# mrjoshuak/go-jpeg2000

Measured on AMD Instinct MI355X. Metric: Mpixels/s encode+decode (4K sRGB, 5-3 lossless), higher is better.
Workload: dtype int32

## Files before the change

### go-jpeg2000_amd/csrc/compact.hip

```cpp
#include "j2k_internal.h"
#include <algorithm>

namespace j2k {

template <bool TWO>
__global__ __launch_bounds__(1024) void scan_lens_kernel(const uint32_t *__restrict__ lens, int n, uint64_t *__restrict__ offs,
                                                         const uint32_t *__restrict__ mels, uint64_t *__restrict__ toffs) {
    __shared__ uint64_t wave_sum[2][16], wave_sum2[2][16];
    const int tid = threadIdx.x, lane = tid & 63, wv = tid >> 6;
    uint64_t carry = 0, carry2 = 0;
    int par = 0;
    for (int base = 0; base < n; base += 8192, par ^= 1) {
        const int i0 = base + tid * 8;
        uint32_t v[8], m[8];
        if (i0 + 8 <= n) {
            const uint4 a = *reinterpret_cast<const uint4 *>(lens + i0), b = *reinterpret_cast<const uint4 *>(lens + i0 + 4);
            v[0] = a.x; v[1] = a.y; v[2] = a.z; v[3] = a.w; v[4] = b.x; v[5] = b.y; v[6] = b.z; v[7] = b.w;
        } else {
#pragma unroll
            for (int k = 0; k < 8; k++) v[k] = (i0 + k < n) ? lens[i0 + k] : 0u;
        }
        if (TWO && i0 + 8 <= n) {
            const uint4 a = *reinterpret_cast<const uint4 *>(mels + i0), b = *reinterpret_cast<const uint4 *>(mels + i0 + 4);
            m[0] = a.x; m[1] = a.y; m[2] = a.z; m[3] = a.w; m[4] = b.x; m[5] = b.y; m[6] = b.z; m[7] = b.w;
        } else {
#pragma unroll
            for (int k = 0; k < 8; k++) m[k] = (TWO && i0 + k < n) ? mels[i0 + k] : 0u;
        }
#pragma unroll
        for (int k = 0; k < 8; k++) m[k] = v[k] ? m[k] : 0u;
        uint64_t t = 0, t2 = 0;
#pragma unroll
        for (int k = 0; k < 8; k++) { t += v[k]; if (TWO) t2 += v[k] - m[k]; }
        uint64_t x = t, x2 = t2;
        for (int o = 1; o < 64; o <<= 1) {
            const uint64_t y = __shfl_up(x, o);
            if (lane >= o) x += y;
            if (TWO) {
                const uint64_t y2 = __shfl_up(x2, o);
                if (lane >= o) x2 += y2;
            }
        }
        if (lane == 63) { wave_sum[par][wv] = x; if (TWO) wave_sum2[par][wv] = x2; }
        __syncthreads();
        uint64_t pre = carry, all = carry, pre2 = carry2, all2 = carry2;
#pragma unroll
        for (int k = 0; k < 16; k++) {
            const uint64_t ws = wave_sum[par][k], ws2 = TWO ? wave_sum2[par][k] : 0;
            if (k < wv) { pre += ws; pre2 += ws2; }
            all += ws; all2 += ws2;
        }
        uint64_t o = pre + x - t, o2 = pre2 + x2 - t2;
#pragma unroll
        for (int k = 0; k < 8; k++) {
            if (i0 + k < n) { offs[i0 + k] = o; if (TWO) toffs[i0 + k] = o2; }
            o += v[k]; o2 += v[k] - m[k];
        }
        carry = all; carry2 = all2;
    }
    if (tid == 0) { offs[n] = carry; if (TWO) toffs[n] = carry2; }
}

__global__ __launch_bounds__(256) void gather_kernel(const BlockJob *__restrict__ jobs, int njobs, const uint8_t *__restrict__ slots,
                                                     const uint32_t *__restrict__ lens, const uint64_t *__restrict__ offs,
                                                     uint8_t *__restrict__ stream, const uint32_t *__restrict__ maglens) {
    const int j = blockIdx.x * 4 + (threadIdx.x >> 6);
    if (j >= njobs) return;
    const int lane = threadIdx.x & 63;
    const uint32_t len = lens[j];
    if (len == 0) return;
    gather_job(jobs[j], slots, stream + offs[j], len, maglens != nullptr, maglens ? maglens[j] : 0u, lane);
}

__global__ __launch_bounds__(256) void gather_scan_kernel(const BlockJob *__restrict__ jobs, int njobs, const uint8_t *__restrict__ slots,
                                                          const uint32_t *__restrict__ lens, uint64_t *__restrict__ offs,
                                                          uint8_t *__restrict__ stream, const uint32_t *__restrict__ maglens) {
    __shared__ uint64_t s_wave[4];
    __shared__ uint32_t s_len[4];
    const int tid = threadIdx.x, wv = tid >> 6, lane = tid & 63;
    const int j0 = blockIdx.x * 4, j = j0 + wv;
    const bool mine = j < njobs;
    const uint32_t len = mine ? lens[j] : 0u;
    const uint32_t mag = (mine && maglens) ? maglens[j] : 0u;
    BlockJob J = jobs[mine ? j : 0];
    uint64_t part = 0;
#pragma unroll
    for (int p = 0; p < 8; p++) {
        const int i0 = 1024 * p + 4 * tid;
        if (i0 + 4 <= j0) {
            const uint4 v = *reinterpret_cast<const uint4 *>(lens + i0);
            part += (uint64_t)v.x + v.y + v.z + v.w;
        } else {
#pragma unroll
            for (int i = 0; i < 3; i++)
                if (i0 + i < j0) part += lens[i0 + i];
        }
    }
#pragma unroll
    for (int o = 32; o > 0; o >>= 1) part += __shfl_xor(part, o);
    if (lane == 0) { s_wave[wv] = part; s_len[wv] = len; }
    __syncthreads();
    uint64_t off = s_wave[0] + s_wave[1] + s_wave[2] + s_wave[3];
#pragma unroll
    for (int k = 0; k < 3; k++)
        if (k < wv) off += s_len[k];
    if (!mine) return;
    if (lane == 0) {
        offs[j] = off;
        if (j == njobs - 1) offs[njobs] = off + len;
    }
    if (len == 0) return;
    gather_job(J, slots, stream + off, len, maglens != nullptr, mag, lane);
}

#define UNPACK_BATCH 16
__host__ __device__ inline size_t pack_a16(size_t x) { return (x + 15) & ~size_t(15); }
struct PackLayout { size_t lens, mag, nb, offs, toffs, payload; };
__host__ __device__ inline PackLayout pack_layout(size_t n) {
    PackLayout L;
    L.lens = 64;
    L.mag = pack_a16(L.lens + 4 * n);
    L.nb = pack_a16(L.mag + 4 * n);
    L.offs = pack_a16(L.nb + n);
    L.toffs = pack_a16(L.offs + 8 * (n + 1));
    L.payload = pack_a16(L.toffs + 8 * (n + 1));
    return L;
}
size_t pack_header_bytes(size_t n) { return pack_layout(n).payload; }

__device__ __forceinline__ uint32_t mel_bytes(const BlockJob &J) {
    const size_t nsamp = (size_t)J.w * J.h;
    return (uint32_t)((nsamp * 2 < 64 ? 64 : nsamp * 2) / 4);
}

__global__ __launch_bounds__(256) void pack_kernel(const BlockJob *__restrict__ jobs, int n, const uint8_t *__restrict__ stream,
                                                   const uint64_t *__restrict__ offs, const uint64_t *__restrict__ toffs,
                                                   const uint32_t *__restrict__ lens, const uint32_t *__restrict__ maglens,
                                                   const uint8_t *__restrict__ numbps, uint8_t *__restrict__ pack) {
    const PackLayout L = pack_layout((size_t)n);
    const int has_mel = maglens != nullptr;
    if (blockIdx.x == 0 && threadIdx.x == 0) {
        uint64_t *h = reinterpret_cast<uint64_t *>(pack);
        h[0] = ((uint64_t)L.payload + toffs[n] + 15) & ~uint64_t(15);
        h[1] = toffs[n];
        reinterpret_cast<uint32_t *>(pack)[4] = (uint32_t)n;
        reinterpret_cast<uint32_t *>(pack)[5] = (uint32_t)has_mel;
    }
    const int j = blockIdx.x * 4 + (threadIdx.x >> 6);
    if (j > n) return;
    const int lane = threadIdx.x & 63;
    const uint64_t off = offs[j], toff = toffs[j];
    if (lane == 0) {
        reinterpret_cast<uint64_t *>(pack + L.offs)[j] = off;
        reinterpret_cast<uint64_t *>(pack + L.toffs)[j] = toff;
    }
    if (j == n) return;
    const uint32_t len = lens[j];
    const uint32_t mag = has_mel ? maglens[j] : len;
    if (lane == 0) {
        reinterpret_cast<uint32_t *>(pack + L.lens)[j] = len;
        reinterpret_cast<uint32_t *>(pack + L.mag)[j] = mag;
        pack[L.nb + j] = numbps[j];
    }
    if (len == 0) return;
    const uint32_t mel = has_mel ? mel_bytes(jobs[j]) : 0u;
    const uint8_t *src = stream + off;
    uint8_t *dst = pack + L.payload + toff;
    copy_bytes(dst, src, mag, lane);
    copy_bytes(dst + mag, src + mag + mel, len - mag - mel, lane);
}
__global__ void mel_table_kernel(const BlockJob *__restrict__ jobs, int n, uint32_t *__restrict__ mels) {
    const int j = blockIdx.x * blockDim.x + threadIdx.x;
    if (j < n) mels[j] = mel_bytes(jobs[j]);
}
struct UnpackBatch {
    const uint8_t *pack[UNPACK_BATCH];
    uint64_t pack_bytes[UNPACK_BATCH];
    uint8_t *stream[UNPACK_BATCH];
    uint64_t *offs[UNPACK_BATCH];
    uint32_t *lens[UNPACK_BATCH];
    uint8_t *numbps[UNPACK_BATCH];
};
__global__ __launch_bounds__(256) void unpack_kernel(const BlockJob *__restrict__ jobs, int n, UnpackBatch B, uint64_t stream_cap,
                                                     int *__restrict__ fault) {
    const uint8_t *__restrict__ pack = B.pack[blockIdx.y];
    uint8_t *__restrict__ stream = B.stream[blockIdx.y];
    uint64_t *__restrict__ offs = B.offs[blockIdx.y];
    uint32_t *__restrict__ lens = B.lens[blockIdx.y];
    uint8_t *__restrict__ numbps = B.numbps[blockIdx.y];
    const PackLayout L = pack_layout((size_t)n);
    const uint64_t avail = B.pack_bytes[blockIdx.y] - L.payload;
    const uint64_t paylen = reinterpret_cast<const uint64_t *>(pack)[1];
    if (reinterpret_cast<const uint32_t *>(pack)[4] != (uint32_t)n || paylen > avail) {
        if (blockIdx.x == 0 && threadIdx.x == 0) atomicMax(fault, 4);
        return;
    }
    const int has_mel = (int)reinterpret_cast<const uint32_t *>(pack)[5];
    const uint64_t *poffs = reinterpret_cast<const uint64_t *>(pack + L.offs);
    const int j = blockIdx.x * 4 + (threadIdx.x >> 6);
    if (j > n) return;
    const int lane = threadIdx.x & 63;
    if (lane == 0) offs[j] = poffs[j];
    if (j == n) return;
    const uint32_t len = reinterpret_cast<const uint32_t *>(pack + L.lens)[j];
    if (lane == 0) { lens[j] = len; numbps[j] = pack[L.nb + j]; }
    if (len == 0) return;
    const uint32_t mag = reinterpret_cast<const uint32_t *>(pack + L.mag)[j];
    const uint32_t mel = has_mel ? mel_bytes(jobs[j]) : 0u;
    const uint64_t toff = reinterpret_cast<const uint64_t *>(pack + L.toffs)[j];
    const uint64_t pj = poffs[j], pn = poffs[n];
    if (mag > len || mel > len - mag || toff > paylen || (uint64_t)(len - mel) > paylen - toff ||
        pn > stream_cap || pj > pn || (uint64_t)len > pn - pj) {
        if (lane == 0) atomicMax(fault, 4);
        return;
    }
    const uint8_t *src = pack + L.payload + toff;
    uint8_t *dst = stream + pj;
    copy_bytes(dst, src, mag, lane);
    zero_run(dst + mag, mel, lane);
    copy_bytes(dst + mag + mel, src + mag, len - mag - mel, lane);
}

hipError_t launch_scan(hipStream_t s, const uint32_t *lens, int njobs, uint64_t *offs, const uint32_t *mels, uint64_t *toffs) {
    if (mels && toffs) hipLaunchKernelGGL(scan_lens_kernel<true>, dim3(1), dim3(1024), 0, s, lens, njobs, offs, mels, toffs);
    else hipLaunchKernelGGL(scan_lens_kernel<false>, dim3(1), dim3(1024), 0, s, lens, njobs, offs, mels, toffs);
    return hipGetLastError();
}
hipError_t launch_pack(hipStream_t s, const BlockJob *jobs, int njobs, const uint8_t *stream, const uint64_t *offs, const uint64_t *toffs,
                       const uint32_t *lens, const uint8_t *numbps, const uint32_t *maglens, uint8_t *pack) {
    hipLaunchKernelGGL(pack_kernel, dim3((njobs + 1 + 3) / 4), dim3(256), 0, s, jobs, njobs, stream, offs, toffs, lens, maglens, numbps, pack);
    return hipGetLastError();
}
hipError_t launch_mel_table(hipStream_t s, const BlockJob *jobs, int njobs, uint32_t *mels) {
    if (njobs <= 0) return hipSuccess;
    hipLaunchKernelGGL(mel_table_kernel, dim3((njobs + 255) / 256), dim3(256), 0, s, jobs, njobs, mels);
    return hipGetLastError();
}
hipError_t launch_unpack(hipStream_t s, const BlockJob *jobs, int njobs, int count, const uint8_t *const *packs, const size_t *pack_bytes,
                         uint8_t *const *streams,
                         size_t stream_cap, uint64_t *const *offs, uint32_t *const *lens, uint8_t *const *numbps, int *fault) {
    for (int c0 = 0; c0 < count; c0 += UNPACK_BATCH) {
        UnpackBatch B{};
        const int m = count - c0 < UNPACK_BATCH ? count - c0 : UNPACK_BATCH;
        for (int i = 0; i < m; i++) {
            B.pack[i] = packs[c0 + i]; B.pack_bytes[i] = (uint64_t)pack_bytes[c0 + i]; B.stream[i] = streams[c0 + i]; B.offs[i] = offs[c0 + i]; B.lens[i] = lens[c0 + i];
            B.numbps[i] = numbps[c0 + i];
        }
        hipLaunchKernelGGL(unpack_kernel, dim3((njobs + 1 + 3) / 4, m), dim3(256), 0, s, jobs, njobs, B, (uint64_t)stream_cap, fault);
    }
    return hipGetLastError();
}

__global__ __launch_bounds__(256) void assemble_tiles_kernel(const uint8_t *__restrict__ stream, const uint64_t *__restrict__ offs,
                                                              const int *__restrict__ job0, int ntiles, int tile_first,
                                                              uint8_t *__restrict__ out, uint64_t *__restrict__ out_len) {
    const int t = blockIdx.x;
    const uint64_t base = offs[job0[0]], o0 = offs[job0[t]], o1 = offs[job0[t + 1]];
    const uint64_t len = o1 - o0;
    uint8_t *dst = out + (o0 - base) + 14ull * (uint64_t)t;
    if (blockIdx.y == 0 && threadIdx.x < 14) {
        const uint32_t idx = (uint32_t)(tile_first + t) & 0xFFFFu, psot = (uint32_t)(14 + len);
        const uint8_t hdr[14] = {0xFF, 0x90, 0x00, 0x0A, (uint8_t)(idx >> 8), (uint8_t)idx, (uint8_t)(psot >> 24), (uint8_t)(psot >> 16),
                                 (uint8_t)(psot >> 8), (uint8_t)psot, 0x00, 0x01, 0xFF, 0x93};
        dst[threadIdx.x] = hdr[threadIdx.x];
    }
    if (out_len && blockIdx.x == 0 && blockIdx.y == 0 && threadIdx.x == 0) *out_len = (offs[job0[ntiles]] - base) + 14ull * (uint64_t)ntiles;
    const uint64_t c0 = (uint64_t)blockIdx.y << 16;
    if (c0 >= len) return;
    const uint32_t n = (uint32_t)(len - c0 < 65536 ? len - c0 : 65536);
    const uint8_t *src = stream + o0 + c0;
    uint8_t *d = dst + 14 + c0;
    const uint32_t head = min(n, (uint32_t)((16 - ((uintptr_t)d & 15)) & 15));
    if (threadIdx.x < head) d[threadIdx.x] = src[threadIdx.x];
    const uint32_t nv = (n - head) >> 4;
    for (uint32_t i = threadIdx.x; i < nv; i += 256) {
        uint4 v;
        __builtin_memcpy(&v, src + head + 16 * (size_t)i, 16);
        *reinterpret_cast<uint4 *>(d + head + 16 * (size_t)i) = v;
    }
    const uint32_t done = head + (nv << 4);
    if (done + threadIdx.x < n) d[done + threadIdx.x] = src[done + threadIdx.x];
}
hipError_t launch_assemble_tiles(hipStream_t s, const uint8_t *stream, const uint64_t *offs, const int *job0, int ntiles, int tile_first,
                                 uint64_t max_tile_bytes, uint8_t *out, uint64_t *out_len) {
    if (ntiles <= 0) return hipSuccess;
    const unsigned chunks = (unsigned)std::max<uint64_t>(1, (max_tile_bytes + 65535) >> 16);
    hipLaunchKernelGGL(assemble_tiles_kernel, dim3(ntiles, chunks), dim3(256), 0, s, stream, offs, job0, ntiles, tile_first, out, out_len);
    return hipGetLastError();
}

hipError_t launch_compact(hipStream_t s, const BlockJob *jobs, int njobs, const uint8_t *slots, const uint32_t *lens,
                          uint64_t *offs, uint8_t *stream, const uint32_t *maglens, const uint32_t *mels, uint64_t *toffs) {
    if (njobs > 0 && njobs <= 8192 && !(mels && toffs) && ((uintptr_t)lens & 15) == 0) {
        hipLaunchKernelGGL(gather_scan_kernel, dim3((njobs + 3) / 4), dim3(256), 0, s, jobs, njobs, slots, lens, offs, stream, maglens);
        return hipGetLastError();
    }
    hipError_t e = launch_scan(s, lens, njobs, offs, mels, toffs);
    if (e != hipSuccess || njobs <= 0) return e;
    hipLaunchKernelGGL(gather_kernel, dim3((njobs + 3) / 4), dim3(256), 0, s, jobs, njobs, slots, lens, offs, stream, maglens);
    return hipGetLastError();
}

}
```

### go-jpeg2000_amd/csrc/j2k_internal.h

```cpp
#pragma once
#include <hip/hip_runtime.h>
#include <stdint.h>
#include <stdlib.h>
#include <algorithm>
#include "../../include/j2kgfx.h"
#include "image_color.h"

namespace j2k {

struct DwtPlane {
    int64_t src_off[3];
    int64_t out_off[3];
    int64_t nxt_off[3];
    int32_t src_stride;
    int32_t w, h;
    int32_t n_next;
    int32_t out_stride;
    int32_t coef_stride;
};

struct DwtJob {
    int32_t plane;
    int32_t col0;
    int32_t prow0;
    int32_t nprow;
};
#define J2K_LINK_UP 0x10000
#define J2K_LINK_DOWN 0x20000

struct BlockJob {
    int64_t src_off;
    int64_t out_off;
    int32_t stride;
    int32_t w, h;
    int32_t band;
};

struct HtUJob {
    BlockJob J;
    int32_t jid;
    int32_t alias_off;
    int32_t nalias;
    int32_t pad_;
};

struct TailPlane {
    int64_t scr_off;
    int64_t coef_off;
    int32_t w, h;
    int32_t nlev;
    int32_t pad_;
};

struct LLPlane {
    int64_t coef_off[3];
    int64_t out_off[3];
    int32_t w, h, coef_stride, out_stride;
    int32_t nc, pad_;
};

struct YccSrc {
    const uint8_t *y, *cb, *cr;
    int64_t ystride, cstride;
    int32_t ratio, pad_;
};

struct LevelLaunch {
    const DwtJob *jobs;
    int njobs;
    const DwtPlane *planes;
    int cpl;
    int vec;
    int ncomp;
    int pf;
    int pix_stride;
    int pix_src;
    long long comp_elems;
    int wg_waves;
    int wg_store;
    const DwtJob *jobs2;
    int njobs2, wg2_waves;
    const DwtPlane *planes1;
    int32_t *nxt1;
    const DwtJob *pjobs;
    int pnjobs, pwaves, pmulti;
    hipEvent_t ev_start, ev_stop;
    YccSrc ycc;
    const int *guard;
    int mallat;
};

hipError_t launch_dwt53_fwd(hipStream_t s, const LevelLaunch &L, const int32_t *src, int32_t *out,
                            int32_t *nxt, int dc_shift);
hipError_t launch_dwt53_inv(hipStream_t s, const LevelLaunch &L, const int32_t *coef, const int32_t *prev,
                            int32_t *dst, int dc_shift, int final_level);
hipError_t launch_dwt53_tail_fwd(hipStream_t s, const TailPlane *planes, int nplanes, size_t lds_bytes, const int32_t *scr,
                                 int32_t *coef, hipEvent_t ev0 = nullptr, hipEvent_t ev1 = nullptr);
hipError_t launch_dwt53_tail_inv(hipStream_t s, const TailPlane *planes, int nplanes, size_t lds_bytes, const int32_t *coef,
                                 int32_t *scr, hipEvent_t ev0 = nullptr, hipEvent_t ev1 = nullptr);

hipError_t launch_dwt53_deep_fwd(hipStream_t s, const DwtJob *jobs, int njobs, const TailPlane *planes, size_t lds_bytes, const int32_t *scr,
                                 int32_t *coef, hipEvent_t ev0, hipEvent_t ev1);
hipError_t launch_dwt53_deep_inv(hipStream_t s, const DwtJob *jobs, int njobs, const TailPlane *planes, size_t lds_bytes, const int32_t *coef,
                                 int32_t *scr, hipEvent_t ev0, hipEvent_t ev1);

hipError_t launch_dwt53_mega_fwd(hipStream_t s, const DwtJob *jobs, int njobs, const TailPlane *tplanes, const DwtPlane *l0planes, size_t lds_bytes,
                                 const int32_t *scr, int32_t *coef, const uint32_t *pix, int32_t *nxt0, int dc_shift, int pix_stride,
                                 hipEvent_t ev0, hipEvent_t ev1);
hipError_t launch_dwt53_mega_inv(hipStream_t s, const DwtJob *jobs, int njobs, const TailPlane *tplanes, const DwtPlane *l0planes, size_t lds_bytes,
                                 const int32_t *coef, int32_t *scr, const int32_t *prev0, uint32_t *pix, int dc_shift, int pix_stride,
                                 hipEvent_t ev0, hipEvent_t ev1);
hipError_t launch_unpack_pixels(hipStream_t s, const uint8_t *pix, size_t stride, int format, int w, int h, int src_max, int dst_max,
                                int32_t *planes);
hipError_t launch_colorspace(hipStream_t s, int cs, int32_t *planes, int ncomp, size_t n, int precision);
hipError_t launch_pack_pixels(hipStream_t s, const int32_t *planes, int ncomp, int precision, int w, int h, uint8_t *pix, size_t stride);
hipError_t launch_pack_pixels_rect(hipStream_t s, const int32_t *planes, int ncomp, int precision, int w, int h, int x0, int y0, int rw, int rh, uint8_t *pix,
                                   size_t stride, const int *guard = nullptr);
hipError_t launch_image_to_rgba8(hipStream_t s, const j2k_image &img, uint32_t *pix, size_t stride_px, int *flag);

hipError_t launch_t2_fill_cbs(hipStream_t s, long n, const uint64_t *offs, const uint32_t *lens, const uint8_t *numbps, int mb, int ht, j2k_t2_dev_cb *cbs, uint64_t *reset = nullptr,
                              const uint8_t *kept = nullptr, const uint32_t *rate = nullptr);
hipError_t launch_t2_encode_tile_parts(hipStream_t s, const j2k_t2_dev_packet *packets, long npackets, const j2k_t2_dev_cb *cbs, uint64_t ncbs, const uint8_t *data,
                                       int sop, int eph, uint8_t *out, uint64_t cap, uint64_t *offs, void *ws, uint64_t *result, const int32_t *ptile,
                                       const int *tile_packet0, int ntiles, int tile_first, uint64_t *tile_offs, int *status, const BlockJob *slot_jobs,
                                       const uint32_t *maglens, int ht, int body_slices);
size_t t2_dev_workspace(long npackets);
hipError_t launch_t2_encode_packets(hipStream_t s, const j2k_t2_dev_packet *packets, long npackets, const j2k_t2_dev_cb *cbs, uint64_t ncbs, const uint8_t *data,
                                    int sop, int eph, int delay_in, uint8_t *out, uint64_t cap, uint64_t *offs, void *ws, uint64_t *result);

__device__ __forceinline__ void copy_bytes(uint8_t *__restrict__ dst, const uint8_t *__restrict__ src, uint32_t n, int lane) {
    const uint32_t head = min(n, (uint32_t)((16 - ((uintptr_t)dst & 15)) & 15));
    if ((uint32_t)lane < head) dst[lane] = src[lane];
    const uint32_t nv = (n - head) >> 4;
    for (uint32_t i = lane; i < nv; i += 64) {
        uint4 v;
        __builtin_memcpy(&v, src + head + 16 * (size_t)i, 16);
        *reinterpret_cast<uint4 *>(dst + head + 16 * (size_t)i) = v;
    }
    const uint32_t done = head + (nv << 4);
    if (done + lane < n) dst[done + lane] = src[done + lane];
}
__device__ __forceinline__ void zero_run(uint8_t *__restrict__ dst, uint32_t n, int lane) {
    const uint32_t head = min(n, (uint32_t)((16 - ((uintptr_t)dst & 15)) & 15));
    if ((uint32_t)lane < head) dst[lane] = 0;
    const uint32_t nv = (n - head) >> 4;
    for (uint32_t i = lane; i < nv; i += 64) *reinterpret_cast<uint4 *>(dst + head + 16 * (size_t)i) = make_uint4(0, 0, 0, 0);
    const uint32_t done = head + (nv << 4);
    if (done + lane < n) dst[done + lane] = 0;
}

__device__ __forceinline__ void gather_job(const BlockJob &J, const uint8_t *__restrict__ slots, uint8_t *__restrict__ dst, uint32_t len,
                                           bool ht, uint32_t mag, int lane) {
    const uint8_t *src = slots + J.out_off;
    if (!ht) {
        copy_bytes(dst, src, len, lane);
        return;
    }
    const size_t nsamp = (size_t)J.w * J.h;
    const uint32_t mel = (uint32_t)((nsamp * 2 < 64 ? 64 : nsamp * 2) / 4);
    copy_bytes(dst, src, mag, lane);
    zero_run(dst + mag, mel, lane);
    copy_bytes(dst + mag + mel, src + mag + mel, len - mag - mel, lane);
}

inline const char *tuning_env(const char *name) {
    static const int on = [] { const char *t = getenv("J2K_TUNING"); return (t && t[0] == '1' && !t[1]) ? 1 : 0; }();
    return on ? getenv(name) : nullptr;
}

#ifdef J2K_DEV
extern int g_dev_skip, g_dev_dup;
inline int dev_reps(int bit) { return (g_dev_skip & bit) ? 0 : ((g_dev_dup & bit) ? 2 : 1); }
#else
constexpr int g_dev_skip = 0;
constexpr int dev_reps(int) { return 1; }
#endif
}
```

Baseline: 78350.

## Replace per-segment byte copies with a single wave-uniform batched gather routine

Adds gather_range, which copies a prefix, zero-fills a middle gap and copies a suffix in one pass. Each lane issues up to six 16-byte global loads before storing them, and a single per-lane byte load/store covers all unaligned edge bytes, replacing the serial head/body/tail loops of copy_bytes and zero_run. The gather_scan prefix sum now issues all lens loads unconditionally before summing, and wave indices are made scalar via readfirstlane. This aims to cut instruction overhead and raise memory-level parallelism for the many small codeblock copies. The cost is more complex edge-case logic built on raw waitcnt intrinsics and address-space casts, which carries a correctness risk.

```diff
diff --git a/go-jpeg2000_amd/csrc/compact.hip b/go-jpeg2000_amd/csrc/compact.hip
--- a/go-jpeg2000_amd/csrc/compact.hip
+++ b/go-jpeg2000_amd/csrc/compact.hip
@@ -64,7 +64,7 @@
 __global__ __launch_bounds__(256) void gather_kernel(const BlockJob *__restrict__ jobs, int njobs, const uint8_t *__restrict__ slots,
                                                      const uint32_t *__restrict__ lens, const uint64_t *__restrict__ offs,
                                                      uint8_t *__restrict__ stream, const uint32_t *__restrict__ maglens) {
-    const int j = blockIdx.x * 4 + (threadIdx.x >> 6);
+    const int j = blockIdx.x * 4 + __builtin_amdgcn_readfirstlane(threadIdx.x >> 6);
     if (j >= njobs) return;
     const int lane = threadIdx.x & 63;
     const uint32_t len = lens[j];
@@ -77,23 +77,24 @@
                                                           uint8_t *__restrict__ stream, const uint32_t *__restrict__ maglens) {
     __shared__ uint64_t s_wave[4];
     __shared__ uint32_t s_len[4];
-    const int tid = threadIdx.x, wv = tid >> 6, lane = tid & 63;
+    const int tid = threadIdx.x, wv = __builtin_amdgcn_readfirstlane(tid >> 6), lane = tid & 63;
     const int j0 = blockIdx.x * 4, j = j0 + wv;
     const bool mine = j < njobs;
     const uint32_t len = mine ? lens[j] : 0u;
     const uint32_t mag = (mine && maglens) ? maglens[j] : 0u;
     BlockJob J = jobs[mine ? j : 0];
     uint64_t part = 0;
-#pragma unroll
-    for (int p = 0; p < 8; p++) {
-        const int i0 = 1024 * p + 4 * tid;
-        if (i0 + 4 <= j0) {
-            const uint4 v = *reinterpret_cast<const uint4 *>(lens + i0);
-            part += (uint64_t)v.x + v.y + v.z + v.w;
-        } else {
-#pragma unroll
-            for (int i = 0; i < 3; i++)
-                if (i0 + i < j0) part += lens[i0 + i];
+    if (j0 > 0) {
+        uint4 v[8];
+#pragma unroll
+        for (int p = 0; p < 8; p++) {
+            const int i0 = 1024 * p + 4 * tid;
+            v[p] = *reinterpret_cast<const uint4 *>(lens + (i0 < j0 ? i0 : 0));
+        }
+#pragma unroll
+        for (int p = 0; p < 8; p++) {
+            const uint64_t sum = (uint64_t)v[p].x + v[p].y + v[p].z + v[p].w;
+            part += 1024 * p + 4 * tid < j0 ? sum : 0;
         }
     }
 #pragma unroll
@@ -166,8 +167,7 @@
     const uint32_t mel = has_mel ? mel_bytes(jobs[j]) : 0u;
     const uint8_t *src = stream + off;
     uint8_t *dst = pack + L.payload + toff;
-    copy_bytes(dst, src, mag, lane);
-    copy_bytes(dst + mag, src + mag + mel, len - mag - mel, lane);
+    gather_range(dst, len - mel, src, mag, 0u, src + mag + mel, lane);
 }
 __global__ void mel_table_kernel(const BlockJob *__restrict__ jobs, int n, uint32_t *__restrict__ mels) {
     const int j = blockIdx.x * blockDim.x + threadIdx.x;
@@ -216,9 +216,7 @@
     }
     const uint8_t *src = pack + L.payload + toff;
     uint8_t *dst = stream + pj;
-    copy_bytes(dst, src, mag, lane);
-    zero_run(dst + mag, mel, lane);
-    copy_bytes(dst + mag + mel, src + mag, len - mag - mel, lane);
+    gather_range(dst, len, src, mag, mel, src + mag, lane);
 }
 
 hipError_t launch_scan(hipStream_t s, const uint32_t *lens, int njobs, uint64_t *offs, const uint32_t *mels, uint64_t *toffs) {
diff --git a/go-jpeg2000_amd/csrc/j2k_internal.h b/go-jpeg2000_amd/csrc/j2k_internal.h
--- a/go-jpeg2000_amd/csrc/j2k_internal.h
+++ b/go-jpeg2000_amd/csrc/j2k_internal.h
@@ -128,39 +128,75 @@
 hipError_t launch_t2_encode_packets(hipStream_t s, const j2k_t2_dev_packet *packets, long npackets, const j2k_t2_dev_cb *cbs, uint64_t ncbs, const uint8_t *data,
                                     int sop, int eph, int delay_in, uint8_t *out, uint64_t cap, uint64_t *offs, void *ws, uint64_t *result);
 
+typedef uint32_t u32x4 __attribute__((ext_vector_type(4)));
+typedef u32x4 __attribute__((aligned(1))) u32x4_any;
+typedef const __attribute__((address_space(1))) u32x4_any *glb_load16;
+typedef __attribute__((address_space(1))) u32x4 *glb_store16;
+typedef const __attribute__((address_space(1))) uint8_t *glb_load1;
+typedef __attribute__((address_space(1))) uint8_t *glb_store1;
+__device__ __forceinline__ void gather_loads_landed(uint32_t &late) {
+    __builtin_amdgcn_s_waitcnt(0x0F70);
+    asm volatile("" : "+v"(late) : : "memory");
+}
+#define GATHER_SLOTS 6
+__device__ __forceinline__ uint32_t wave_value(uint32_t x) { return (uint32_t)__builtin_amdgcn_readfirstlane((int)x); }
+__device__ __forceinline__ uint64_t wave_value(const void *p) {
+    const uint64_t u = (uint64_t)(uintptr_t)p;
+    return (uint64_t)wave_value((uint32_t)(u >> 32)) << 32 | wave_value((uint32_t)u);
+}
+__device__ __forceinline__ void gather_range(uint8_t *__restrict__ dst_, uint32_t n, const uint8_t *__restrict__ srca_, uint32_t a, uint32_t z,
+                                             const uint8_t *__restrict__ srcc_, int lane) {
+    const uint64_t dst = wave_value(dst_), srca = wave_value(srca_), srcc = wave_value(srcc_);
+    n = wave_value(n);
+    if (n == 0) return;
+    a = min(wave_value(a), n);
+    z = min(wave_value(z), n - a);
+    const uint32_t d0 = (uint32_t)dst & 15, qa = d0 + a, qz = qa + z, qe = d0 + n;
+    const uint64_t base = dst - d0;
+    const uint32_t pa0 = (d0 + 15) >> 4, pz0 = (qa + 15) >> 4, pc0 = (qz + 15) >> 4;
+    const uint32_t pa1 = max(qa >> 4, pa0), pz1 = max(qz >> 4, pz0), pc1 = max(qe >> 4, pc0);
+    const uint32_t na = pa1 - pa0, nl = na + (pc1 - pc0);
+    const int g = lane >> 4;
+    const uint32_t c0 = 0, c1 = qa >> 4, c2 = qz >> 4, c3 = (qe - 1) >> 4;
+    const uint32_t bp = g == 0 ? c0 : g == 1 ? c1 : g == 2 ? c2 : c3;
+    const bool again = (g > 0 && bp == c0) || (g > 1 && bp == c1) || (g > 2 && bp == c2);
+    const bool whole = (bp >= pa0 && bp < pa1) || (bp >= pz0 && bp < pz1) || (bp >= pc0 && bp < pc1);
+    const uint32_t bq = 16 * bp + (uint32_t)(lane & 15);
+    const bool bput = !again && !whole && bq >= d0 && bq < qe, bload = bput && (bq < qa || bq >= qz);
+    const uint64_t bfrom = !bload ? (a ? srca : n - a - z ? srcc : dst) : bq < qa ? srca + (bq - d0) : srcc + (bq - qz);
+    uint32_t bval = *(glb_load1)bfrom;
+    uint32_t s0 = 0;
+    do {
+        u32x4 v[GATHER_SLOTS];
+#pragma unroll
+        for (int i = 0; i < GATHER_SLOTS; i++) {
+            if (s0 + 64 * i >= nl) break;
+            const uint32_t s = s0 + 64 * i + (uint32_t)lane, sc = s < nl ? s : s0;
+            v[i] = *(glb_load16)(sc < na ? srca + ((uint64_t)16 * (pa0 + sc) - d0) : srcc + ((uint64_t)16 * (pc0 + (sc - na)) - qz));
+        }
+        gather_loads_landed(bval);
+        if (s0 == 0 && bput) *(glb_store1)(base + bq) = bload ? (uint8_t)bval : (uint8_t)0;
+#pragma unroll
+        for (int i = 0; i < GATHER_SLOTS; i++) {
+            const uint32_t s = s0 + 64 * i + (uint32_t)lane;
+            if (s < nl) *(glb_store16)(base + (uint64_t)16 * (s < na ? pa0 + s : pc0 + (s - na))) = v[i];
+        }
+        s0 += 64 * GATHER_SLOTS;
+    } while (s0 < nl);
+    const u32x4 zero = {0, 0, 0, 0};
+    for (uint32_t p = pz0 + (uint32_t)lane; p < pz1; p += 64) *(glb_store16)(base + (uint64_t)16 * p) = zero;
+}
 __device__ __forceinline__ void copy_bytes(uint8_t *__restrict__ dst, const uint8_t *__restrict__ src, uint32_t n, int lane) {
-    const uint32_t head = min(n, (uint32_t)((16 - ((uintptr_t)dst & 15)) & 15));
-    if ((uint32_t)lane < head) dst[lane] = src[lane];
-    const uint32_t nv = (n - head) >> 4;
-    for (uint32_t i = lane; i < nv; i += 64) {
-        uint4 v;
-        __builtin_memcpy(&v, src + head + 16 * (size_t)i, 16);
-        *reinterpret_cast<uint4 *>(dst + head + 16 * (size_t)i) = v;
-    }
-    const uint32_t done = head + (nv << 4);
-    if (done + lane < n) dst[done + lane] = src[done + lane];
-}
-__device__ __forceinline__ void zero_run(uint8_t *__restrict__ dst, uint32_t n, int lane) {
-    const uint32_t head = min(n, (uint32_t)((16 - ((uintptr_t)dst & 15)) & 15));
-    if ((uint32_t)lane < head) dst[lane] = 0;
-    const uint32_t nv = (n - head) >> 4;
-    for (uint32_t i = lane; i < nv; i += 64) *reinterpret_cast<uint4 *>(dst + head + 16 * (size_t)i) = make_uint4(0, 0, 0, 0);
-    const uint32_t done = head + (nv << 4);
-    if (done + lane < n) dst[done + lane] = 0;
+    gather_range(dst, n, src, n, 0, src, lane);
 }
 
 __device__ __forceinline__ void gather_job(const BlockJob &J, const uint8_t *__restrict__ slots, uint8_t *__restrict__ dst, uint32_t len,
                                            bool ht, uint32_t mag, int lane) {
     const uint8_t *src = slots + J.out_off;
-    if (!ht) {
-        copy_bytes(dst, src, len, lane);
-        return;
-    }
     const size_t nsamp = (size_t)J.w * J.h;
-    const uint32_t mel = (uint32_t)((nsamp * 2 < 64 ? 64 : nsamp * 2) / 4);
-    copy_bytes(dst, src, mag, lane);
-    zero_run(dst + mag, mel, lane);
-    copy_bytes(dst + mag + mel, src + mag + mel, len - mag - mel, lane);
+    const uint32_t mel = ht ? (uint32_t)((nsamp * 2 < 64 ? 64 : nsamp * 2) / 4) : 0u;
+    if (!ht) mag = len;
+    gather_range(dst, len, src, mag, mel, src + mag + mel, lane);
 }
 
 inline const char *tuning_env(const char *name) {
```

After: 79070 (median of 6 runs). About the same (+0.9%).
